# JoHof/lungmask

Measured on AMD Instinct MI355X. Metric: CT slices/sec (whole node), R231 512x512 volume, higher is better.
Workload: dtype f16x3-split (hi/lo f16 operands, f32 accumulate; fp32-class)

## Files before the change

### lungmask_amd/csrc/lm_platform.h

```cpp
#pragma once
#ifdef LM_EMU_BUILD
#include "hip_emu.h"
#else
#include <hip/hip_runtime.h>
#define LM_LAUNCH(kernel, grid, block, smem, stream, ...) \
    hipLaunchKernelGGL(kernel, (grid), (block), (smem), (stream), __VA_ARGS__)
#define LM_DYN_SMEM(name) extern __shared__ __attribute__((aligned(16))) char name[]
typedef float lm_f32x16 __attribute__((ext_vector_type(16)));
typedef float lm_f32x4 __attribute__((ext_vector_type(4)));
#endif
#include <cstdint>
#ifdef LM_EMU_BUILD
#define LM_IS_GPU_BUILD 0
#else
#define LM_IS_GPU_BUILD 1
#endif

#ifndef LM_EMU_BUILD
typedef _Float16 lm_h16;
typedef _Float16 lm_h16x8 __attribute__((ext_vector_type(8)));
__device__ __forceinline__ float lm_h2f(lm_h16 h) { return (float)h; }
__device__ __forceinline__ lm_h16 lm_f2h(float f) { return (lm_h16)f; }
#endif

// ... 208 lines not shown
    lm_h16 l[4] = {lm_f2h(v0 - lm_h2f(h[0])), lm_f2h(v1 - lm_h2f(h[1])), lm_f2h(v2 - lm_h2f(h[2])), lm_f2h(v3 - lm_h2f(h[3]))};
    memcpy(hi, h, 8);
    memcpy(lo, l, 8);
#else
    typedef _Float16 h4 __attribute__((ext_vector_type(4)));
    typedef float f4 __attribute__((ext_vector_type(4)));
    const f4 v = {v0, v1, v2, v3};
    const h4 h = __builtin_convertvector(v, h4);
    __builtin_memcpy(hi, &h, 8);
    unsigned l01, l23;
    asm("v_fma_mixlo_f16 %0, %1, 1.0, -%2 op_sel_hi:[0,0,1]" : "=v"(l01) : "v"(v0), "v"(hi->x));
    asm("v_fma_mixhi_f16 %0, %1, 1.0, -%2 op_sel:[0,0,1] op_sel_hi:[0,0,1]" : "+v"(l01) : "v"(v1), "v"(hi->x));
    asm("v_fma_mixlo_f16 %0, %1, 1.0, -%2 op_sel_hi:[0,0,1]" : "=v"(l23) : "v"(v2), "v"(hi->y));
    asm("v_fma_mixhi_f16 %0, %1, 1.0, -%2 op_sel:[0,0,1] op_sel_hi:[0,0,1]" : "+v"(l23) : "v"(v3), "v"(hi->y));
    lo->x = l01;
    lo->y = l23;
#endif
}
__device__ __forceinline__ unsigned lm_pk_absmax_u16(unsigned acc, unsigned two_halves) {
    const unsigned m = two_halves & 0x7fff7fffu;
#ifdef LM_EMU_BUILD
    const unsigned lo = (acc & 0xffffu) > (m & 0xffffu) ? (acc & 0xffffu) : (m & 0xffffu);
    const unsigned hi = (acc >> 16) > (m >> 16) ? (acc >> 16) : (m >> 16);
    return lo | (hi << 16);
#else
    typedef unsigned short u16x2 __attribute__((ext_vector_type(2)));
    u16x2 a, b;
    __builtin_memcpy(&a, &acc, 4);
    __builtin_memcpy(&b, &m, 4);
    a = __builtin_elementwise_max(a, b);
    unsigned r;
    __builtin_memcpy(&r, &a, 4);
    return r;
#endif
}
__device__ __forceinline__ bool lm_pk_out_of_f16_guard(unsigned acc) { return (acc & 0xffffu) >= 0x7800u || (acc >> 16) >= 0x7800u; }

__device__ __forceinline__ void lm_unsplit4(uint2 hi, uint2 lo, float* out) {
#ifdef LM_EMU_BUILD
    lm_h16 h[4], l[4];
    memcpy(h, &hi, 8);
    memcpy(l, &lo, 8);
    for (int k = 0; k < 4; ++k) out[k] = lm_h2f(l[k]) + lm_h2f(h[k]);
#else
    typedef _Float16 h4 __attribute__((ext_vector_type(4)));
    typedef float f4 __attribute__((ext_vector_type(4)));
    h4 h, l;
    __builtin_memcpy(&h, &hi, 8);
    __builtin_memcpy(&l, &lo, 8);
    const f4 r = __builtin_convertvector(l, f4) + __builtin_convertvector(h, f4);
    out[0] = r[0];
    out[1] = r[1];
    out[2] = r[2];
    out[3] = r[3];
#endif
}

#ifdef LM_EMU_BUILD
typedef float lm_f32x2 __attribute__((vector_size(8)));
#else
typedef float lm_f32x2 __attribute__((ext_vector_type(2)));
#endif

template <int K>
__device__ __forceinline__ void lm_fmac_rowbcast(float& acc, float w, float x) {
#ifdef LM_EMU_BUILD
    acc = fmaf(__shfl(w, ((int)(lm_emu::linear_tid() & 63) & ~15) | K), x, acc);
#else
    asm("v_fmac_f32_dpp %0, %1, %2 row_newbcast:%3 row_mask:0xf bank_mask:0xf" : "+v"(acc) : "v"(w), "v"(x), "n"(K));
#endif
}
template <int K>
__device__ __forceinline__ float lm_mov_rowbcast(float w) {
#ifdef LM_EMU_BUILD
    return __shfl(w, ((int)(lm_emu::linear_tid() & 63) & ~15) | K);
#else
    float r = 0.f;
    asm("v_mov_b32_dpp %0, %1 row_newbcast:%2 row_mask:0xf bank_mask:0xf" : "+v"(r) : "v"(w), "n"(K));
    return r;
#endif
}

#ifdef LM_EMU_BUILD
#define LM_SCHED_FENCE() \
    do {                 \
    } while (0)
#else
#define LM_SCHED_FENCE() __builtin_amdgcn_sched_barrier(0)
#endif
#ifdef LM_EMU_BUILD
#define LM_LDS_WAIT6(N, a, b, c, d, e, f) \
    do {                                  \
    } while (0)
#define LM_LDS_READ128(dst, ptr, OFF) (dst) = *reinterpret_cast<const lm_h16x8*>(reinterpret_cast<const char*>(ptr) + (OFF))
#define LM_LDS_WAIT8(N, a, b, c, d, e, f, g, h) \
    do {                                        \
    } while (0)
#define LM_LDS_WAIT5(N, a, b, c, d, e) \
    do {                               \
    } while (0)
#define LM_LDS_WAIT2(N, a, b) \
    do {                      \
    } while (0)
#define LM_LDS_WAIT1(N, a) \
    do {                   \
    } while (0)
#define LM_LDS_WRITE2_64(ptr, lo8, hi8)                                  \
    do {                                                                 \
        *reinterpret_cast<uint2*>(reinterpret_cast<char*>(ptr)) = (lo8); \
        *reinterpret_cast<uint2*>(reinterpret_cast<char*>(ptr) + 16) = (hi8); \
    } while (0)
#else
typedef unsigned lm_u32x2 __attribute__((ext_vector_type(2)));
#define LM_LDS_WRITE2_64(ptr, lo8, hi8)                                                                                      \
    do {                                                                                                                     \
        const lm_u32x2 d0_ = {(lo8).x, (lo8).y}, d1_ = {(hi8).x, (hi8).y};                                                   \
        asm volatile("ds_write2_b64 %0, %1, %2 offset1:2"                                                                    \
                     :                                                                                                       \
                     : "v"((unsigned)(size_t)(__attribute__((address_space(3))) char*)(ptr)), "v"(d0_), "v"(d1_)            \
                     : "memory");                                                                                            \
    } while (0)
#define LM_LDS_WAIT2(N, a, b)                                                                \
    do {                                                                                     \
        asm volatile("s_waitcnt lgkmcnt(%2)" : "+v"(a), "+v"(b) : "i"(N) : "memory");        \
        __builtin_amdgcn_sched_barrier(0);                                                   \
    } while (0)
#define LM_LDS_WAIT1(N, a)                                                                   \
    do {                                                                                     \
        asm volatile("s_waitcnt lgkmcnt(%1)" : "+v"(a) : "i"(N) : "memory");                 \
        __builtin_amdgcn_sched_barrier(0);                                                   \
    } while (0)
#define LM_LDS_WAIT5(N, a, b, c, d, e)                                                                            \
    do {                                                                                                          \
        asm volatile("s_waitcnt lgkmcnt(%5)" : "+v"(a), "+v"(b), "+v"(c), "+v"(d), "+v"(e) : "i"(N) : "memory");  \
        __builtin_amdgcn_sched_barrier(0);                                                                        \
    } while (0)
#define LM_LDS_WAIT6(N, a, b, c, d, e, f)                                                                         \
    do {                                                                                                          \
        asm volatile("s_waitcnt lgkmcnt(%6)" : "+v"(a), "+v"(b), "+v"(c), "+v"(d), "+v"(e), "+v"(f) : "i"(N) : "memory"); \
        __builtin_amdgcn_sched_barrier(0);                                                                        \
    } while (0)
#define LM_LDS_READ128(dst, ptr, OFF)                                                                             \
    asm volatile("ds_read_b128 %0, %1 offset:%2"                                                                  \
                 : "=v"(dst)                                                                                      \
                 : "v"((unsigned)(size_t)(__attribute__((address_space(3))) const char*)(ptr)), "i"(OFF)          \
                 : "memory")
#define LM_LDS_WAIT8(N, a, b, c, d, e, f, g, h)                                                                   \
    do {                                                                                                          \
        asm volatile("s_waitcnt lgkmcnt(%8)"                                                                      \
                     : "+v"(a), "+v"(b), "+v"(c), "+v"(d), "+v"(e), "+v"(f), "+v"(g), "+v"(h)                     \
                     : "i"(N)                                                                                     \
                     : "memory");                                                                                 \
        __builtin_amdgcn_sched_barrier(0);                                                                        \
    } while (0)
#endif
```

### lungmask_amd/csrc/nn_kernels_h3.hip

```cpp
#include <cstdlib>

#include "nn_kernels.h"

#if defined(LM_H3_TRACE) || defined(LM_H3_TIMELINE)
__device__ unsigned* lm_h3_trace_ptr = nullptr;
#endif

namespace lm {

namespace {

constexpr int TH = 16, TW = 16, TN = 64, KC = 16;

typedef uint2 __attribute__((may_alias)) uint2_a;
typedef uint4 __attribute__((may_alias)) uint4_a;

__device__ __forceinline__ void split_store4(char* group_base, int half_off_bytes, float v0, float v1, float v2, float v3) {
    uint2 ph, plo;
    lm_split4(v0, v1, v2, v3, &ph, &plo);
    *reinterpret_cast<uint2*>(group_base + half_off_bytes) = ph;
    *reinterpret_cast<uint2*>(group_base + 16 + half_off_bytes) = plo;
}

template <int TAPS>
struct H3Smem {
    static constexpr int HALO = (TAPS == 9) ? 1 : 0;
    static constexpr int PW = TW + 2 * HALO, PH = TH + 2 * HALO;
    static constexpr int A_ROWS = PH * PW;
    static constexpr int W_ROWS = TAPS * TN;
    static constexpr int ROW_BYTES = KC * 4;
    static constexpr int A_BYTES = ((A_ROWS * ROW_BYTES + 1023) / 1024) * 1024;
    static constexpr int W_BYTES = W_ROWS * ROW_BYTES;
    static constexpr int BYTES = A_BYTES + W_BYTES;
};

}

template <int TAPS>
__global__ __launch_bounds__(256, 2) void conv_igemm_h3(ConvParamsH3 p) {
    using SM = H3Smem<TAPS>;
    constexpr int HALO = SM::HALO, PW = SM::PW, A_ROWS = SM::A_ROWS, W_ROWS = SM::W_ROWS;
    LM_DYN_SMEM(smem);
    char* As = smem;
    char* Ws = smem + SM::A_BYTES;

    const int tid = threadIdx.x, lane = tid & 63, wave = tid >> 6;
    const int tiles_x = (p.W + TW - 1) / TW, tiles_y = (p.H + TH - 1) / TH;
    int t = blockIdx.x;
    const int tx = t % tiles_x;
    t /= tiles_x;
    const int ty = t % tiles_y;
    const int b = t / tiles_y;
    const int x0 = tx * TW, y0 = ty * TH, n0 = blockIdx.y * TN;

    lm_f32x16 accm[2][2];
#pragma unroll
    for (int i = 0; i < 2; ++i)
#pragma unroll
        for (int j = 0; j < 2; ++j)
#pragma unroll
            for (int r = 0; r < 16; ++r) {
                accm[i][j][r] = 0.f;
            }

    const int li = lane & 31, kb = lane >> 5;
    const int pr = li >> 4, pc = li & 15;
    const char* __restrict__ in_b = p.in + ((size_t)b * p.H * p.W * p.in_cstride + p.in_coff) * 4;
    const size_t w_row_bytes = (size_t)p.Cin * 4;

    for (int c0 = 0; c0 < p.Cin; c0 += KC) {
        __syncthreads();
        for (int piece = wave; piece * 64 < A_ROWS * 4; piece += 4) {
            const int idx = piece * 64 + lane;
            if (idx < A_ROWS * 4) {
                const int row = idx >> 2, ls = (idx & 3) ^ ((row >> 2) & 3);
                const int py = row / PW, px = row - py * PW;
                const int gy = y0 + py - HALO, gx = x0 + px - HALO;
                const char* src = p.zeros;
                if (gy >= 0 && gy < p.H && gx >= 0 && gx < p.W)
                    src = in_b + ((size_t)gy * p.W + gx) * p.in_cstride * 4 + (size_t)((c0 >> 3) + (ls >> 1)) * 32 + (ls & 1) * 16;
                lm_global_load_lds16(src, As + piece * 1024);
            }
        }
// ... 30 lines not shown
                for (int nt = 0; nt < 2; ++nt) {
                    accm[mt][nt] = lm_mfma_f32_32x32x16_f16(whi[mt], ahi[nt], accm[mt][nt]);
                    accm[mt][nt] = lm_mfma_f32_32x32x16_f16(whi[mt], alo[nt], accm[mt][nt]);
                    accm[mt][nt] = lm_mfma_f32_32x32x16_f16(wlo[mt], ahi[nt], accm[mt][nt]);
                }
        }
    }

    const bool bn = p.bn_s != nullptr;
    float amax = 0.f;
    const int Hp = p.H >> 1, Wp = p.W >> 1;
#pragma unroll
    for (int nt = 0; nt < 2; ++nt) {
        const int y = y0 + 4 * wave + 2 * nt + pr, x = x0 + pc;
        const bool inside = y < p.H && x < p.W;
        char* orow = p.out + ((((size_t)b * p.H + y) * p.W + x) * p.out_cstride + p.out_coff) * 4;
        const bool pool_lane = p.pool != nullptr && pr == 0 && (pc & 1) == 0;
        char* prow = p.pool ? p.pool + ((((size_t)b * Hp + (y >> 1)) * Wp + (x >> 1)) * p.pool_cstride + p.pool_coff) * 4 : nullptr;
#pragma unroll
        for (int mt = 0; mt < 2; ++mt) {
#pragma unroll
            for (int g = 0; g < 4; ++g) {
                const int cb = n0 + 32 * mt + 8 * g + 4 * kb;
                float4 bias = *reinterpret_cast<const float4*>(p.bias + cb);
                if (TAPS == 9 && p.border_corr != nullptr) {
                    const int mask = (y == 0 ? 1 : 0) | (y == p.H - 1 ? 2 : 0) | (x == 0 ? 4 : 0) | (x == p.W - 1 ? 8 : 0);
                    const float4 c = *reinterpret_cast<const float4*>(p.border_corr + (size_t)mask * p.Cout + cb);
                    bias.x -= c.x;
                    bias.y -= c.y;
                    bias.z -= c.z;
                    bias.w -= c.w;
                }
                float v[4];
                v[0] = fmaf(accm[mt][nt][4 * g + 0], p.acc_scale, bias.x);
                v[1] = fmaf(accm[mt][nt][4 * g + 1], p.acc_scale, bias.y);
                v[2] = fmaf(accm[mt][nt][4 * g + 2], p.acc_scale, bias.z);
                v[3] = fmaf(accm[mt][nt][4 * g + 3], p.acc_scale, bias.w);
                if (bn) {
                    const float4 s = *reinterpret_cast<const float4*>(p.bn_s + cb);
                    const float4 sh = *reinterpret_cast<const float4*>(p.bn_t + cb);
                    v[0] = fmaf(fmaxf(v[0], 0.f), s.x, sh.x);
                    v[1] = fmaf(fmaxf(v[1], 0.f), s.y, sh.y);
                    v[2] = fmaf(fmaxf(v[2], 0.f), s.z, sh.z);
                    v[3] = fmaf(fmaxf(v[3], 0.f), s.w, sh.w);
                }
                amax = fmaxf(fmaxf(amax, fabsf(v[0])), fmaxf(fmaxf(fabsf(v[1]), fabsf(v[2])), fabsf(v[3])));
                const int grp = cb >> 3;
                if (inside) split_store4(orow + (size_t)grp * 32, (cb & 7) * 2, v[0], v[1], v[2], v[3]);
                if (p.pool != nullptr) {
                    float q[4];
#pragma unroll
                    for (int k = 0; k < 4; ++k) {
                        const float h = v[k] + __shfl_xor(v[k], 1);
                        q[k] = 0.25f * (h + __shfl_xor(h, 16));
                    }
                    if (pool_lane && y + 1 < p.H && x + 1 < p.W) split_store4(prow + (size_t)grp * 32, (cb & 7) * 2, q[0], q[1], q[2], q[3]);
                }
            }
        }
    }
    if (p.range_flag != nullptr && !(amax < kF16Guard)) atomicOr(p.range_flag, 1u);
}

namespace {
template <int TAPS, bool G16>
struct H3WSmem {
    static constexpr int HALO = (TAPS == 9) ? 1 : 0;
    static constexpr int TWW = G16 ? 16 : 32;
    static constexpr int NSL = G16 ? 2 : 1;
    static constexpr int PW = TWW + 2 * HALO, PH = TH + 2 * HALO;
    static constexpr int SL_ROWS = PH * PW;
    static constexpr int A_ROWS = NSL * SL_ROWS;
    static constexpr int NTSTEP = G16 ? 2 : 1;
    static constexpr int W_ROWS = TAPS * TN;
    static constexpr int A_PIECES = (A_ROWS * 4 + 63) / 64, W_PIECES = W_ROWS * 4 / 64;
    static constexpr int A_BYTES = A_PIECES * 1024, W_BYTES = W_PIECES * 1024;
    static constexpr int BUF_BYTES = A_BYTES + W_BYTES;
    static constexpr int NW = 8;
    static constexpr int A_PER_WAVE = (A_PIECES + NW - 1) / NW, W_PER_WAVE = (W_PIECES + NW - 1) / NW;
};

__device__ __forceinline__ float4 as_float4(const lm_h16x8& v) {
    float4 r;
    memcpy(&r, &v, 16);
    return r;
}
}

#define H3P_READS(F, AS, DY, DX)                                                              \
    do {                                                                                      \
        const int a_lo_ = a_off[DX] ^ 16;                                                     \
        LM_LDS_READ128(F[4], (AS) + a_off[DX], (DY) * ROWB);                                  \
        LM_LDS_READ128(F[5], (AS) + a_lo_, (DY) * ROWB);                                      \
        LM_LDS_READ128(F[6], (AS) + a_off[DX], ((DY) + NTSTEP) * ROWB);                       \
        LM_LDS_READ128(F[7], (AS) + a_lo_, ((DY) + NTSTEP) * ROWB);                           \
        LM_LDS_READ128(F[0], (AS) + w_off, (3 * (DY) + (DX)) * (TN * 64));                    \
        LM_LDS_READ128(F[1], (AS) + w_off, (3 * (DY) + (DX)) * (TN * 64) + 2048);             \
        LM_LDS_READ128(F[2], (AS) + w_off_lo, (3 * (DY) + (DX)) * (TN * 64));                 \
        LM_LDS_READ128(F[3], (AS) + w_off_lo, (3 * (DY) + (DX)) * (TN * 64) + 2048);          \
    } while (0)
#define H3P_MFMA3(F, I0, I1, I2)                                                              \
    do {                                                                                      \
        H3P_MFMA1(F, I0);                                                                     \
        H3P_MFMA1(F, I1);                                                                     \
        H3P_MFMA1(F, I2);                                                                     \
    } while (0)
#define H3P_MFMA1(F, I)                                                                                                           \
    accm[((I) >> 1) & 1][(I) & 1] = lm_mfma_f32_32x32x16_f16(F[((I) < 8 ? 0 : 2) + (((I) >> 1) & 1)],                             \
                                                            F[4 + 2 * ((I) & 1) + (((I) >> 2) == 1 ? 1 : 0)], accm[((I) >> 1) & 1][(I) & 1])
#define H3P_MFMA2(F, I0, I1) \
    do {                     \
        H3P_MFMA1(F, I0);    \
        H3P_MFMA1(F, I1);    \
    } while (0)
#define H3P_MFMAS(F, PS)       \
    do {                       \
        prod_step(PS, 0);      \
        H3P_MFMA2(F, 0, 1);    \
        prod_step(PS, 1);      \
        H3P_MFMA2(F, 2, 3);    \
        prod_step(PS, 2);      \
        H3P_MFMA2(F, 4, 5);    \
        prod_step(PS, 3);      \
        H3P_MFMA2(F, 6, 7);    \
        prod_step(PS, 4);      \
        H3P_MFMA2(F, 8, 9);    \
        prod_step(PS, 5);      \
        H3P_MFMA2(F, 10, 11);  \
    } while (0)
#define H3P_MFMAS_D(F, K0, PS) \
    do {                       \
        prod_step(PS, 0);      \
        H3P_MFMA2(F, 0, 1);    \
        prod_step(PS, 1);      \
        H3P_MFMA1(F, 2);       \
        dma_slot((K0) + 0);    \
        H3P_MFMA1(F, 3);       \
        prod_step(PS, 2);      \
        H3P_MFMA2(F, 4, 5);    \
        dma_slot((K0) + 1);    \
        prod_step(PS, 3);      \
        H3P_MFMA2(F, 6, 7);    \
        prod_step(PS, 4);      \
        H3P_MFMA1(F, 8);       \
        dma_slot((K0) + 2);    \
        H3P_MFMA1(F, 9);       \
        prod_step(PS, 5);      \
        H3P_MFMA2(F, 10, 11);  \
        dma_slot((K0) + 3);    \
    } while (0)
#define H3P_WAITF(N, F) LM_LDS_WAIT8(N, F[0], F[1], F[2], F[3], F[4], F[5], F[6], F[7])
#define H3P_STEP(FC, FN, AS, NDY, NDX, PS) \
    do {                                   \
        H3P_READS(FN, AS, NDY, NDX);       \
        H3P_WAITF(8, FC);                  \
        H3P_MFMAS(FC, PS);                 \
    } while (0)
#define H3P_STEP_D(FC, FN, AS, NDY, NDX, K0, PS) \
    do {                                         \
        H3P_READS(FN, AS, NDY, NDX);             \
        H3P_WAITF(8, FC);                        \
        H3P_MFMAS_D(FC, K0, PS);                 \
    } while (0)
#define H3P_CHUNK_STEPS(FA, FB, AS)             \
    do {                                        \
        H3P_STEP_D(FA, FB, AS, 0, 1, 0, 1);     \
        H3P_STEP_D(FB, FA, AS, 0, 2, 4, 2);     \
        H3P_STEP_D(FA, FB, AS, 1, 0, 8, 3);     \
        H3P_STEP(FB, FA, AS, 1, 1, 4);          \
        H3P_STEP(FA, FB, AS, 1, 2, 5);          \
        H3P_STEP(FB, FA, AS, 2, 0, 6);          \
        H3P_STEP(FA, FB, AS, 2, 1, 7);          \
        H3P_STEP(FB, FA, AS, 2, 2, 8);          \
    } while (0)

#define H3P_EPI_READS(E, CL) LM_LDS_READ128(E[0], ep + (CL) * 4, 0)
#define H3P_EPI_WAIT(NEXT, E) LM_LDS_WAIT1((NEXT) ? 1 : 0, E[0])
#define H3P_EPI_CL(MG) (32 * ((MG) >> 2) + 8 * ((MG) & 3) + 4 * kb)

namespace {
constexpr int FC_PW = 36, FC_PH = 20, FC_PATCH = FC_PW * FC_PH;
constexpr int FC_CONST = 9 * 64 + 64 + 64;
constexpr int FC_ROW = 68;
static_assert(10 * FC_ROW <= FC_CONST, "the DPP producer's constant table");
constexpr int FC_TASKS = 18 * 34 * 2;

}

template <int TAPS, bool G16, int HEAD = 0, int PROD = 0, bool KS = false>
__global__ __launch_bounds__(512) void conv_igemm_h3p(ConvParamsH3 p, int n_ptiles, int n_items, int xcd_order) {
    using SM = H3WSmem<TAPS, G16>;
    static_assert(!KS || (TAPS == 9 && HEAD == 0 && PROD == 0), "the split-K instantiation is the plain 3x3 form");
    constexpr bool KSPLIT = TAPS == 1 || KS;
    static_assert(PROD == 0 || (TAPS == 9 && !G16 && HEAD == 0), "the loader-side producers belong to the 32-wide 3x3 form");
    constexpr int HALO = SM::HALO, PW = SM::PW, TWW = SM::TWW, NW = SM::NW, ROWB = PW * 64, NTSTEP = SM::NTSTEP;
    constexpr int ASWZ = (G16 && TAPS == 9) ? 1 : 2;
    constexpr int HSTR = 144;
    constexpr int STAGE_BYTES = NW * 64 * HSTR;
    constexpr int SUB = TAPS == 1 ? 2 : 1;
    constexpr int STAGE_EXTRA = STAGE_BYTES <= SUB * SM::BUF_BYTES ? 0 : STAGE_BYTES;
    __shared__ __attribute__((aligned(1024))) char lds[2 * SUB * SM::BUF_BYTES + STAGE_EXTRA];
    __shared__ __attribute__((aligned(16))) float epi[2][3][TN];
    __shared__ __attribute__((aligned(16))) float hw[HEAD ? kMaxClasses * 64 + kMaxClasses : 4];
    __shared__ __attribute__((aligned(16))) float fcx[PROD == 1 ? 2 * FC_PATCH : 4];
    __shared__ __attribute__((aligned(16))) float fcc[PROD == 1 ? FC_CONST : 4];

    const int tid = threadIdx.x, lane = tid & 63, wave = lm_uniform(tid >> 6);
    const int li = lane & 31, kb = lane >> 5;
    const int wsl = G16 ? (wave >> 2) : 0;
    const int wrow = G16 ? 4 * (wave & 3) + (li >> 4) : 2 * wave;
    const int wcol = G16 ? (li & 15) : li;

    int a_off[TAPS == 9 ? 3 : 1];
#pragma unroll
    for (int dx = 0; dx < (TAPS == 9 ? 3 : 1); ++dx) {
        const int px = wcol + dx;
        a_off[dx] = (wsl * SM::SL_ROWS + wrow * PW + px) * 64 + ((2 * kb) ^ ((px >> ASWZ) & 3)) * 16;
    }
    const int w_off = SM::A_BYTES + li * 64 + ((2 * kb) ^ ((li >> 2) & 3)) * 16;
    const int w_off_lo = w_off ^ 16;

    unsigned relA[SM::A_PER_WAVE];
    int pyx[SM::A_PER_WAVE];
#pragma unroll
    for (int j = 0; j < SM::A_PER_WAVE; ++j) {
        const int piece = wave + NW * j, idx = piece * 64 + lane;
        pyx[j] = -1;
        relA[j] = 0;
        if (PROD != 1 && piece < SM::A_PIECES && idx < SM::A_ROWS * 4) {
            const int row = idx >> 2;
            const int sl = row / SM::SL_ROWS, rr = row - sl * SM::SL_ROWS;
            const int py = rr / PW, px = rr - py * PW;
            const int ls = (idx & 3) ^ ((px >> ASWZ) & 3);
            relA[j] = (unsigned)(((sl * p.H + py) * p.W + px) * p.in_cstride * 4 + (ls >> 1) * 32 + (ls & 1) * 16);
            pyx[j] = py | (px << 8) | (sl << 16);
        }
    }
    unsigned voffW;
    {
        const int idx = wave * 64 + lane;
        const int row = idx >> 2, ls = (idx & 3) ^ ((row >> 2) & 3);
        const int tap = row / TN, n = row - tap * TN;
        voffW = (unsigned)((tap * p.Cout + n) * p.Cin * 4 + (ls >> 1) * 32 + (ls & 1) * 16);
    }
    const unsigned w_piece_stride = (unsigned)(NW * 64 / 4 / TN) * (unsigned)p.Cout * (unsigned)p.Cin * 4u;
    const unsigned slice_bytes = (unsigned)p.H * (unsigned)p.W * (unsigned)p.in_cstride * 4u;
    const lm_rsrc rsrcA = PROD == 1 ? lm_make_rsrc(p.fc_x, (size_t)p.B * p.H * p.W * 4)
                                    : lm_make_rsrc(p.in + (size_t)p.in_coff * 4, (size_t)p.B * slice_bytes - (size_t)p.in_coff * 4);
    const lm_rsrc rsrcW = lm_make_rsrc(p.w, (size_t)TAPS * p.Cout * p.Cin * 4);
    const int tiles_x = p.W / TWW;
    const int nchunks = p.Cin / KC / ((KSPLIT && p.ksplit > 1) ? p.ksplit : 1);
    constexpr bool bn = TAPS == 9;

    const int n_ct = p.Cout / TN;
    const int tiles_y = (p.H + TH - 1) / TH;
    const bool pow2 = ((n_ct & (n_ct - 1)) | (tiles_x & (tiles_x - 1)) | (tiles_y & (tiles_y - 1))) == 0;
    const int sh_ct = 31 - __clz(n_ct), sh_tx = 31 - __clz(tiles_x), sh_ty = 31 - __clz(tiles_y);
    const int ksplit = (KSPLIT && p.ksplit > 1) ? p.ksplit : 1;
    auto decode = [&](int it, int& b, int& y0, int& x0, int& n0, int& kc) -> bool {
        int ct, pt;
        if (xcd_order) {
// ... 333 lines not shown
                        } else {
                            H3P_EPI_WAIT(false, ec[mg & 1]);
                        }
                        const float4 bias = as_float4(ec[mg & 1][0]);
                        float bb[4] = {bias.x, bias.y, bias.z, bias.w};
                        if (border) {
                            const float4 c = cb[mg];
                            bb[0] -= c.x;
                            bb[1] -= c.y;
                            bb[2] -= c.z;
                            bb[3] -= c.w;
                        }
                        float v[4];
#pragma unroll
                        for (int k = 0; k < 4; ++k) {
                            float t = fmaf(accm[mt][nt][4 * g4 + k], p.acc_scale, bb[k]);
                            if (bn) t = fmaxf(t, 0.f);
                            v[k] = t;
                        }
#pragma unroll
                        for (int k = 0; k < 4; ++k) vv[mg][k] = v[k];
                    }
                    float best = 0.f;
                    int arg = 0;
                    float lgs[HEAD == 2 ? kMaxClasses : 1];
                    auto logit = [&](int c) __attribute__((always_inline)) -> float {
                        float sq[8];
#pragma unroll
                        for (int q = 0; q < 8; ++q) {
                            const float4 w4 = *reinterpret_cast<const float4*>(&hw[c * 64 + 8 * q + 4 * kb]);
                            float s0 = fmaf(vv[q][0], w4.x, 0.f);
                            s0 = fmaf(vv[q][1], w4.y, s0);
                            s0 = fmaf(vv[q][2], w4.z, s0);
                            s0 = fmaf(vv[q][3], w4.w, s0);
                            float s1 = __shfl_xor(s0, 32);
                            s1 = fmaf(vv[q][0], w4.x, s1);
                            s1 = fmaf(vv[q][1], w4.y, s1);
                            s1 = fmaf(vv[q][2], w4.z, s1);
                            s1 = fmaf(vv[q][3], w4.w, s1);
                            sq[q] = s1;
                        }
                        return (((sq[0] + sq[4]) + (sq[2] + sq[6])) + ((sq[1] + sq[5]) + (sq[3] + sq[7]))) + hw[kMaxClasses * 64 + c];
                    };
                    if constexpr (HEAD == 2) {
#pragma unroll
                        for (int c = 0; c < kMaxClasses; ++c) {
                            if (c < p.head_C) {
                                const float lg = logit(c);
                                lgs[c] = lg;
                                if (c == 0 || lg > best) {
                                    best = lg;
                                    arg = c;
                                }
                            }
                        }
                    } else {
#pragma unroll 1
                        for (int c = 0; c < p.head_C; ++c) {
                            const float lg = logit(c);
                            if (c == 0 || lg > best) {
                                best = lg;
                                arg = c;
                            }
                        }
                    }
                    if (tile_ok && kb == 1) p.head_labels[((size_t)bs * p.H + yl) * p.W + x0 + li] = (uint8_t)arg;
                    if constexpr (HEAD == 2) {
                        float se = 0.f;
#pragma unroll
                        for (int c = 0; c < kMaxClasses; ++c)
                            if (c < p.head_C) se += expf(lgs[c] - best);
                        const float lse = best + logf(se);
                        if (tile_ok && kb == 1) {
                            const size_t HW = (size_t)p.H * p.W, yx = (size_t)yl * p.W + x0 + li;
#pragma unroll
                            for (int c = 0; c < kMaxClasses; ++c)
                                if (c < p.head_C) p.head_logp[((size_t)bs * p.head_C + c) * HW + yx] = lgs[c] - lse;
                        }
                    }
                }
            } else {
            int yl2[2], bmask2[2];
            bool ok2[2], border2[2];
            char* obase[2];
#pragma unroll
            for (int nt = 0; nt < 2; ++nt) {
                yl2[nt] = G16 ? yb + 2 * nt + (li >> 4) : yb + nt;
                ok2[nt] = bs < p.B && (G16 ? yb + 2 * nt + 1 < p.H : yb + nt < p.H);
                const int xl = G16 ? wcol : x0 + li;
                bmask2[nt] = (yl2[nt] == 0 ? 1 : 0) | (yl2[nt] == p.H - 1 ? 2 : 0) | (xl == 0 ? 4 : 0) | (xl == p.W - 1 ? 8 : 0);
                border2[nt] = TAPS == 9 && p.border_corr != nullptr && __any(bmask2[nt] != 0);
                const int y_first = G16 ? yb + 2 * nt : yb + nt;
                obase[nt] = p.out + ((((size_t)bs * p.H + y_first) * p.W + x0) * p.out_cstride + p.out_coff + n0) * 4;
            }
#pragma unroll
            for (int mt = 0; mt < 2; ++mt) {
                float4 cb[2][2];
                auto load_cb = [&](int g4) __attribute__((always_inline)) {
#pragma unroll
                    for (int nt = 0; nt < 2; ++nt)
                        if (border2[nt])
                            cb[g4 & 1][nt] = *reinterpret_cast<const float4*>(p.border_corr + (size_t)bmask2[nt] * p.Cout + n0 + H3P_EPI_CL(4 * mt + g4));
                };
                load_cb(0);
                float qs[4][4];
                lm_h16x8 ec[2][3];
                H3P_EPI_READS(ec[0], H3P_EPI_CL(4 * mt));
#pragma unroll
                for (int g4 = 0; g4 < 4; ++g4) {
                    const int mg = 4 * mt + g4;
                    const int cl = H3P_EPI_CL(mg);
                    if (g4 + 1 < 4) {
                        H3P_EPI_READS(ec[(g4 + 1) & 1], H3P_EPI_CL(mg + 1));
                        H3P_EPI_WAIT(true, ec[g4 & 1]);
                    } else {
                        H3P_EPI_WAIT(false, ec[g4 & 1]);
                    }
                    const float4 bias = as_float4(ec[g4 & 1][0]);
                    if (g4 + 1 < 4) load_cb(g4 + 1);
                    float v[2][4];
#pragma unroll
                    for (int nt = 0; nt < 2; ++nt) {
                        float bb[4] = {bias.x, bias.y, bias.z, bias.w};
                        if (border2[nt]) {
                            const float4 c = cb[g4 & 1][nt];
                            bb[0] -= c.x;
                            bb[1] -= c.y;
                            bb[2] -= c.z;
                            bb[3] -= c.w;
                        }
#pragma unroll
                        for (int k = 0; k < 4; ++k) {
                            float t = fmaf(accm[mt][nt][4 * g4 + k], p.acc_scale, bb[k]);
                            if (bn) t = fmaxf(t, 0.f);
                            v[nt][k] = t;
                        }
                        uint2 ph, plo;
                        lm_split4(v[nt][0], v[nt][1], v[nt][2], v[nt][3], &ph, &plo);
                        gmax = lm_pk_absmax_u16(lm_pk_absmax_u16(gmax, ph.x), ph.y);
                        char* d = hstage + (nt * 32 + li) * HSTR + ((cl & 31) >> 3) * 32 + (cl & 7) * 2;
                        *reinterpret_cast<uint2_a*>(d) = ph;
                        *reinterpret_cast<uint2_a*>(d + 16) = plo;
                        if (G16 && p.pool != nullptr) {
                            float q[4];
#pragma unroll
                            for (int k = 0; k < 4; ++k) {
                                const float h = v[nt][k] + __shfl_xor(v[nt][k], 16);
                                q[k] = 0.25f * (h + __shfl_xor(h, 1));
                            }
                            if (ok2[nt] && (li & 17) == 0) {
                                const int cg = n0 + cl;
                                char* prow = p.pool + ((((size_t)bs * Hp + (yl2[nt] >> 1)) * Wp + (wcol >> 1)) * p.pool_cstride + p.pool_coff) * 4;
                                split_store4(prow + (size_t)(cg >> 3) * 32, (cg & 7) * 2, q[0], q[1], q[2], q[3]);
                            }
                        }
                    }
                    if (!G16 && p.pool != nullptr) {
#pragma unroll
                        for (int k = 0; k < 4; ++k) {
                            const float pl = v[0][k] + v[1][k];
                            qs[g4][k] = 0.25f * (pl + lm_lane_xor1(pl));
                        }
                    }
                }
                LM_TRACE_SUB(5);
                lm_wave_lds_fence();
#pragma unroll
                for (int i = 0; i < 8; ++i) {
                    const int q = i * 64 + lane, px = q >> 3, part = q & 7;
                    if (ok2[i >> 2]) {
                        const uint4 val = *reinterpret_cast<const uint4_a*>(hstage + px * HSTR + part * 16);
                        char* dst = obase[i >> 2] + (size_t)(px & 31) * p.out_cstride * 4 + mt * 128 + part * 16;
                        if (p.stream_out) lm_store16_stream(dst, val);
                        else *reinterpret_cast<uint4_a*>(dst) = val;
                    }
                }
                lm_wave_lds_fence();
                LM_TRACE_SUB(6);
                if (!G16 && p.pool != nullptr) {
#pragma unroll
                    for (int g4 = 0; g4 < 4; ++g4) {
                        const int cl = H3P_EPI_CL(4 * mt + g4);
                        uint2 ph, plo;
                        lm_split4(qs[g4][0], qs[g4][1], qs[g4][2], qs[g4][3], &ph, &plo);
                        if ((li & 1) == 0) {
                            char* d = hstage + (li >> 1) * HSTR + ((cl & 31) >> 3) * 32 + (cl & 7) * 2;
                            *reinterpret_cast<uint2_a*>(d) = ph;
                            *reinterpret_cast<uint2_a*>(d + 16) = plo;
                        }
                    }
                    lm_wave_lds_fence();
                    if (bs < p.B && yb + 1 < p.H) {
                        char* prow = p.pool + ((((size_t)bs * Hp + (yb >> 1)) * Wp + (x0 >> 1)) * p.pool_cstride + p.pool_coff + n0) * 4;
#pragma unroll
                        for (int i = 0; i < 2; ++i) {
                            const int q = i * 64 + lane, px = q >> 3, part = q & 7;
                            const uint4 val = *reinterpret_cast<const uint4_a*>(hstage + px * HSTR + part * 16);
                            *reinterpret_cast<uint4_a*>(prow + (size_t)px * p.pool_cstride * 4 + mt * 128 + part * 16) = val;
                        }
                    }
                    lm_wave_lds_fence();
                }
            }
            }
            if (p.range_flag != nullptr && lm_pk_out_of_f16_guard(gmax)) atomicOr(p.range_flag, 1u);
        }
        LM_TRACE_MARK(3);
        if (!have_next) break;
        it = nit;
        b = nb;
        y0 = ny0;
        x0 = nx0;
        n0 = nn0;
        kc0 = nkc0;
#pragma unroll
        for (int j = 0; j < SM::A_PER_WAVE; ++j) voffC[j] = voffN[j];
        epar ^= 1;
        lm_barrier_lds();
        LM_TRACE_MARK(4);
    }
    if (PROD != 0 && p.range_flag != nullptr && lm_pk_out_of_f16_guard(pr_max)) atomicOr(p.range_flag, 1u);
    LM_TRACE_FLUSH();
}

static bool h3_persistent_ok(const ConvParamsH3& p, int taps) {
    static const bool wide_ok = [] { const char* e = getenv("LM_H3_FALLBACK"); return !(e && e[0] == '1'); }();
    const size_t slice_bytes = (size_t)p.H * p.W * p.in_cstride * 4;
    return wide_ok && (p.W % 32 == 0 || p.W == 16) && (p.Cin / KC) % (taps == 1 ? 4 : 2) == 0 && 2 * slice_bytes < 0x7fffffffull &&
           (size_t)taps * p.Cout * p.Cin * 4 < 0x7fffffffull && (p.bn_s != nullptr) == (taps == 9);
}

template <int TAPS>
static hipError_t launch_conv_h3_t(const ConvParamsH3& p, hipStream_t stream) {
    if (p.Cin % KC != 0 || p.Cout % TN != 0 || (p.in_cstride & 7) || (p.in_coff & 7) || (p.out_cstride & 7) || (p.out_coff & 7)) return hipErrorInvalidValue;
    if (p.pool != nullptr && (((p.H | p.W) & 1) || (p.pool_cstride & 7) || (p.pool_coff & 7))) return hipErrorInvalidValue;
    if (h3_persistent_ok(p, TAPS)) {
        const bool g16 = p.W == 16;
        static const int order_env = [] { const char* e = getenv("LM_H3_ORDER"); return e ? atoi(e) : -1; }();
        static const int n_cu = [] {
            int dev = 0, n = 256;
            if (hipGetDevice(&dev) == hipSuccess) (void)hipDeviceGetAttribute(&n, hipDeviceAttributeMultiprocessorCount, dev);
            return n > 0 ? n : 256;
        }();
        const size_t slice_bytes = (size_t)p.H * p.W * p.in_cstride * 4;
        const int max_b = std::max(2, (int)(0x7fffffffull / slice_bytes) & ~1);
        for (int b0 = 0; b0 < p.B; b0 += max_b) {
            ConvParamsH3 pd = p;
            pd.B = std::min(max_b, p.B - b0);
            pd.in = p.in + (size_t)b0 * slice_bytes;
            pd.out = p.out + (size_t)b0 * p.H * p.W * p.out_cstride * 4;
            if (p.pool) pd.pool = p.pool + (size_t)b0 * (p.H / 2) * (p.W / 2) * p.pool_cstride * 4;
            if (p.head_labels) pd.head_labels = p.head_labels + (size_t)b0 * p.H * p.W;
            if (p.head_logp) pd.head_logp = p.head_logp + (size_t)b0 * p.head_C * p.H * p.W;
            if (p.fc_x) pd.fc_x = p.fc_x + (size_t)b0 * p.H * p.W;
            const int n_ptiles = g16 ? ((p.H + TH - 1) / TH) * ((pd.B + 1) / 2) : (p.W / 32) * ((p.H + TH - 1) / TH) * pd.B;
            const int n_ct = p.Cout / TN;
            const int ks = p.ksplit > 1 ? p.ksplit : 1;
            const int xcd_order = ks > 1 ? 0 : (order_env >= 0 ? order_env : (n_ct >= 2 && n_ptiles >= 64 ? 1 : 0));
            const int n_items = xcd_order ? 8 * ((n_ptiles + 7) / 8) * n_ct : n_ptiles * n_ct * ks;
            const unsigned blocks = (unsigned)std::min(n_items, n_cu);
            if (TAPS == 9 && ks > 1) {
                if (g16) LM_LAUNCH((conv_igemm_h3p<9, true, 0, 0, true>), dim3(blocks), dim3(512), 0, stream, pd, n_ptiles, n_items, xcd_order);
                else LM_LAUNCH((conv_igemm_h3p<9, false, 0, 0, true>), dim3(blocks), dim3(512), 0, stream, pd, n_ptiles, n_items, xcd_order);
            } else if (g16)
                LM_LAUNCH((conv_igemm_h3p<TAPS, true>), dim3(blocks), dim3(512), 0, stream, pd, n_ptiles, n_items, xcd_order);
            else if (TAPS == 9 && pd.head_labels != nullptr && pd.head_logp != nullptr)
                LM_LAUNCH((conv_igemm_h3p<9, false, 2>), dim3(blocks), dim3(512), 0, stream, pd, n_ptiles, n_items, xcd_order);
            else if (TAPS == 9 && pd.head_labels != nullptr)
                LM_LAUNCH((conv_igemm_h3p<9, false, 1>), dim3(blocks), dim3(512), 0, stream, pd, n_ptiles, n_items, xcd_order);
            else if (TAPS == 9 && pd.fc_x != nullptr)
                LM_LAUNCH((conv_igemm_h3p<9, false, 0, 1>), dim3(blocks), dim3(512), 0, stream, pd, n_ptiles, n_items, xcd_order);
            else
                LM_LAUNCH((conv_igemm_h3p<TAPS, false>), dim3(blocks), dim3(512), 0, stream, pd, n_ptiles, n_items, xcd_order);
            const hipError_t err = hipGetLastError();
            if (err != hipSuccess) return err;
        }
        return hipSuccess;
    }
    const int tiles = ((p.W + TW - 1) / TW) * ((p.H + TH - 1) / TH);
    dim3 grid((unsigned)(tiles * p.B), (unsigned)(p.Cout / TN));
    LM_LAUNCH((conv_igemm_h3<TAPS>), grid, dim3(256), (H3Smem<TAPS>::BYTES), stream, p);
    return hipGetLastError();
}

bool conv3x3_h3_can_fuse_head(const ConvParamsH3& p) {
// ... 361 lines not shown
```

Before: 4479.

## Batch epilogue LDS reads and hoist border-correction and pool stores out of loop

Restructures the conv epilogue. The output write-back now issues eight ds_read_b128 up front with explicit partial lgkmcnt waits and uses precomputed per-lane row pointers. The stream/non-stream choice is resolved at compile time instead of per store. Border-correction vectors are loaded once for all 8 channel groups before the mt loop, and the pooled-output staging/store is merged into a single pass after both mt iterations. This cuts LDS latency stalls, per-iteration global loads and address arithmetic, at the cost of more live registers (cb[8][2], qs[8][4]), which may lower occupancy or cause spills.

```diff
diff --git a/lungmask_amd/csrc/lm_platform.h b/lungmask_amd/csrc/lm_platform.h
--- a/lungmask_amd/csrc/lm_platform.h
+++ b/lungmask_amd/csrc/lm_platform.h
@@ -314,6 +314,13 @@
 }
 
 #ifdef LM_EMU_BUILD
+#define LM_ASM_TAG(T) \
+    do {              \
+    } while (0)
+#else
+#define LM_ASM_TAG(T) asm volatile("; " T ::: "memory")
+#endif
+#ifdef LM_EMU_BUILD
 #define LM_SCHED_FENCE() \
     do {                 \
     } while (0)
@@ -330,6 +337,9 @@
     } while (0)
 #define LM_LDS_WAIT5(N, a, b, c, d, e) \
     do {                               \
+    } while (0)
+#define LM_LDS_WAIT4(N, a, b, c, d) \
+    do {                            \
     } while (0)
 #define LM_LDS_WAIT2(N, a, b) \
     do {                      \
@@ -361,6 +371,11 @@
     do {                                                                                     \
         asm volatile("s_waitcnt lgkmcnt(%1)" : "+v"(a) : "i"(N) : "memory");                 \
         __builtin_amdgcn_sched_barrier(0);                                                   \
+    } while (0)
+#define LM_LDS_WAIT4(N, a, b, c, d)                                                                               \
+    do {                                                                                                          \
+        asm volatile("s_waitcnt lgkmcnt(%4)" : "+v"(a), "+v"(b), "+v"(c), "+v"(d) : "i"(N) : "memory");           \
+        __builtin_amdgcn_sched_barrier(0);                                                                        \
     } while (0)
 #define LM_LDS_WAIT5(N, a, b, c, d, e)                                                                            \
     do {                                                                                                          \
diff --git a/lungmask_amd/csrc/nn_kernels_h3.hip b/lungmask_amd/csrc/nn_kernels_h3.hip
--- a/lungmask_amd/csrc/nn_kernels_h3.hip
+++ b/lungmask_amd/csrc/nn_kernels_h3.hip
@@ -1,4 +1,5 @@
 #include <cstdlib>
+#include <type_traits>
 
 #include "nn_kernels.h"
 
@@ -195,6 +196,11 @@
 
 __device__ __forceinline__ float4 as_float4(const lm_h16x8& v) {
     float4 r;
+    memcpy(&r, &v, 16);
+    return r;
+}
+__device__ __forceinline__ uint4 as_uint4(const lm_h16x8& v) {
+    uint4 r;
     memcpy(&r, &v, 16);
     return r;
 }
@@ -290,6 +296,8 @@
 #define H3P_EPI_READS(E, CL) LM_LDS_READ128(E[0], ep + (CL) * 4, 0)
 #define H3P_EPI_WAIT(NEXT, E) LM_LDS_WAIT1((NEXT) ? 1 : 0, E[0])
 #define H3P_EPI_CL(MG) (32 * ((MG) >> 2) + 8 * ((MG) & 3) + 4 * kb)
+#define H3P_OUT_READ(L, BASE, I) LM_LDS_READ128(L[I], BASE, (I) * 8 * HSTR)
+#define H3P_OUT_WAIT4(N, L, I) LM_LDS_WAIT4(N, L[(I)], L[(I) + 1], L[(I) + 2], L[(I) + 3])
 
 namespace {
 constexpr int FC_PW = 36, FC_PH = 20, FC_PATCH = FC_PW * FC_PH;
@@ -789,7 +797,7 @@
             } else {
             int yl2[2], bmask2[2];
             bool ok2[2], border2[2];
-            char* obase[2];
+            char* orow[2];
 #pragma unroll
             for (int nt = 0; nt < 2; ++nt) {
                 yl2[nt] = G16 ? yb + 2 * nt + (li >> 4) : yb + nt;
@@ -798,19 +806,63 @@
                 bmask2[nt] = (yl2[nt] == 0 ? 1 : 0) | (yl2[nt] == p.H - 1 ? 2 : 0) | (xl == 0 ? 4 : 0) | (xl == p.W - 1 ? 8 : 0);
                 border2[nt] = TAPS == 9 && p.border_corr != nullptr && __any(bmask2[nt] != 0);
                 const int y_first = G16 ? yb + 2 * nt : yb + nt;
-                obase[nt] = p.out + ((((size_t)bs * p.H + y_first) * p.W + x0) * p.out_cstride + p.out_coff + n0) * 4;
-            }
+                orow[nt] = p.out + ((((size_t)bs * p.H + y_first) * p.W + x0 + (lane >> 3)) * p.out_cstride + p.out_coff + n0) * 4 + (lane & 7) * 16;
+            }
+            const size_t ostep = (size_t)p.out_cstride * 32;
+            const char* const hread = hstage + (lane >> 3) * HSTR + (lane & 7) * 16;
+            lm_f32x4 cb[TAPS == 9 ? 8 : 1][2];
+            if constexpr (TAPS == 9) {
+                if (border2[0] || border2[1]) {
+#pragma unroll
+                    for (int mg = 0; mg < 8; ++mg)
+#pragma unroll
+                        for (int nt = 0; nt < 2; ++nt)
+                            cb[mg][nt] = *reinterpret_cast<const lm_f32x4*>(p.border_corr + (size_t)bmask2[nt] * p.Cout + n0 + H3P_EPI_CL(mg));
+#pragma unroll
+                    for (int mg = 0; mg < 8; ++mg)
+#pragma unroll
+                        for (int nt = 0; nt < 2; ++nt) LM_PIN(cb[mg][nt]);
+                } else {
+#pragma unroll
+                    for (int mg = 0; mg < 8; ++mg)
+#pragma unroll
+                        for (int nt = 0; nt < 2; ++nt) cb[mg][nt] = lm_f32x4{0.f, 0.f, 0.f, 0.f};
+                }
+            }
+            auto store_lines = [&](int mt, auto stream) __attribute__((always_inline)) {
+                lm_h16x8 ln[8];
+                LM_ASM_TAG("LM_STORE_OUT_BEGIN");
+                H3P_OUT_READ(ln, hread, 0);
+                H3P_OUT_READ(ln, hread, 1);
+                H3P_OUT_READ(ln, hread, 2);
+                H3P_OUT_READ(ln, hread, 3);
+                H3P_OUT_READ(ln, hread, 4);
+                H3P_OUT_READ(ln, hread, 5);
+                H3P_OUT_READ(ln, hread, 6);
+                H3P_OUT_READ(ln, hread, 7);
+                H3P_OUT_WAIT4(4, ln, 0);
+                if (ok2[0]) {
+#pragma unroll
+                    for (int i = 0; i < 4; ++i) {
+                        char* dst = orow[0] + i * ostep + mt * 128;
+                        if constexpr (decltype(stream)::value) lm_store16_stream(dst, as_uint4(ln[i]));
+                        else *reinterpret_cast<uint4_a*>(dst) = as_uint4(ln[i]);
+                    }
+                }
+                H3P_OUT_WAIT4(0, ln, 4);
+                if (ok2[1]) {
+#pragma unroll
+                    for (int i = 0; i < 4; ++i) {
+                        char* dst = orow[1] + i * ostep + mt * 128;
+                        if constexpr (decltype(stream)::value) lm_store16_stream(dst, as_uint4(ln[4 + i]));
+                        else *reinterpret_cast<uint4_a*>(dst) = as_uint4(ln[4 + i]);
+                    }
+                }
+                LM_ASM_TAG("LM_STORE_OUT_END");
+            };
+            float qs[8][4];
 #pragma unroll
             for (int mt = 0; mt < 2; ++mt) {
-                float4 cb[2][2];
-                auto load_cb = [&](int g4) __attribute__((always_inline)) {
-#pragma unroll
-                    for (int nt = 0; nt < 2; ++nt)
-                        if (border2[nt])
-                            cb[g4 & 1][nt] = *reinterpret_cast<const float4*>(p.border_corr + (size_t)bmask2[nt] * p.Cout + n0 + H3P_EPI_CL(4 * mt + g4));
-                };
-                load_cb(0);
-                float qs[4][4];
                 lm_h16x8 ec[2][3];
                 H3P_EPI_READS(ec[0], H3P_EPI_CL(4 * mt));
 #pragma unroll
@@ -824,17 +876,16 @@
                         H3P_EPI_WAIT(false, ec[g4 & 1]);
                     }
                     const float4 bias = as_float4(ec[g4 & 1][0]);
-                    if (g4 + 1 < 4) load_cb(g4 + 1);
                     float v[2][4];
 #pragma unroll
                     for (int nt = 0; nt < 2; ++nt) {
                         float bb[4] = {bias.x, bias.y, bias.z, bias.w};
-                        if (border2[nt]) {
-                            const float4 c = cb[g4 & 1][nt];
-                            bb[0] -= c.x;
-                            bb[1] -= c.y;
-                            bb[2] -= c.z;
-                            bb[3] -= c.w;
+                        if constexpr (TAPS == 9) {
+                            const lm_f32x4 c = cb[mg][nt];
+                            bb[0] -= c[0];
+                            bb[1] -= c[1];
+                            bb[2] -= c[2];
+                            bb[3] -= c[3];
                         }
 #pragma unroll
                         for (int k = 0; k < 4; ++k) {
@@ -855,6 +906,8 @@
                                 const float h = v[nt][k] + __shfl_xor(v[nt][k], 16);
                                 q[k] = 0.25f * (h + __shfl_xor(h, 1));
                             }
+#pragma unroll
+                            for (int k = 0; k < 4; ++k) LM_PIN(q[k]);
                             if (ok2[nt] && (li & 17) == 0) {
                                 const int cg = n0 + cl;
                                 char* prow = p.pool + ((((size_t)bs * Hp + (yl2[nt] >> 1)) * Wp + (wcol >> 1)) * p.pool_cstride + p.pool_coff) * 4;
@@ -866,48 +919,46 @@
 #pragma unroll
                         for (int k = 0; k < 4; ++k) {
                             const float pl = v[0][k] + v[1][k];
-                            qs[g4][k] = 0.25f * (pl + lm_lane_xor1(pl));
+                            qs[mg][k] = 0.25f * (pl + lm_lane_xor1(pl));
                         }
                     }
                 }
                 LM_TRACE_SUB(5);
                 lm_wave_lds_fence();
-#pragma unroll
-                for (int i = 0; i < 8; ++i) {
-                    const int q = i * 64 + lane, px = q >> 3, part = q & 7;
-                    if (ok2[i >> 2]) {
-                        const uint4 val = *reinterpret_cast<const uint4_a*>(hstage + px * HSTR + part * 16);
-                        char* dst = obase[i >> 2] + (size_t)(px & 31) * p.out_cstride * 4 + mt * 128 + part * 16;
-                        if (p.stream_out) lm_store16_stream(dst, val);
-                        else *reinterpret_cast<uint4_a*>(dst) = val;
-                    }
-                }
+                if (p.stream_out) store_lines(mt, std::true_type{});
+                else store_lines(mt, std::false_type{});
                 lm_wave_lds_fence();
                 LM_TRACE_SUB(6);
-                if (!G16 && p.pool != nullptr) {
-#pragma unroll
-                    for (int g4 = 0; g4 < 4; ++g4) {
-                        const int cl = H3P_EPI_CL(4 * mt + g4);
-                        uint2 ph, plo;
-                        lm_split4(qs[g4][0], qs[g4][1], qs[g4][2], qs[g4][3], &ph, &plo);
-                        if ((li & 1) == 0) {
-                            char* d = hstage + (li >> 1) * HSTR + ((cl & 31) >> 3) * 32 + (cl & 7) * 2;
-                            *reinterpret_cast<uint2_a*>(d) = ph;
-                            *reinterpret_cast<uint2_a*>(d + 16) = plo;
-                        }
+            }
+            if (!G16 && p.pool != nullptr) {
+#pragma unroll
+                for (int mg = 0; mg < 8; ++mg) {
+                    const int cl = H3P_EPI_CL(mg);
+                    uint2 ph, plo;
+                    lm_split4(qs[mg][0], qs[mg][1], qs[mg][2], qs[mg][3], &ph, &plo);
+                    if ((li & 1) == 0) {
+                        char* d = hstage + ((mg >> 2) * 16 + (li >> 1)) * HSTR + ((cl & 31) >> 3) * 32 + (cl & 7) * 2;
+                        *reinterpret_cast<uint2_a*>(d) = ph;
+                        *reinterpret_cast<uint2_a*>(d + 16) = plo;
                     }
-                    lm_wave_lds_fence();
-                    if (bs < p.B && yb + 1 < p.H) {
-                        char* prow = p.pool + ((((size_t)bs * Hp + (yb >> 1)) * Wp + (x0 >> 1)) * p.pool_cstride + p.pool_coff + n0) * 4;
-#pragma unroll
-                        for (int i = 0; i < 2; ++i) {
-                            const int q = i * 64 + lane, px = q >> 3, part = q & 7;
-                            const uint4 val = *reinterpret_cast<const uint4_a*>(hstage + px * HSTR + part * 16);
-                            *reinterpret_cast<uint4_a*>(prow + (size_t)px * p.pool_cstride * 4 + mt * 128 + part * 16) = val;
-                        }
-                    }
-                    lm_wave_lds_fence();
-                }
+                }
+                lm_wave_lds_fence();
+                lm_h16x8 ln[4];
+                LM_ASM_TAG("LM_STORE_OUT_BEGIN");
+                H3P_OUT_READ(ln, hread, 0);
+                H3P_OUT_READ(ln, hread, 1);
+                H3P_OUT_READ(ln, hread, 2);
+                H3P_OUT_READ(ln, hread, 3);
+                H3P_OUT_WAIT4(0, ln, 0);
+                if (bs < p.B && yb + 1 < p.H) {
+                    char* prow = p.pool + ((((size_t)bs * Hp + (yb >> 1)) * Wp + (x0 >> 1) + (lane >> 3)) * p.pool_cstride + p.pool_coff + n0) * 4 + (lane & 7) * 16;
+                    const size_t pstep = (size_t)p.pool_cstride * 32;
+#pragma unroll
+                    for (int i = 0; i < 4; ++i)
+                        *reinterpret_cast<uint4_a*>(prow + (i & 1) * pstep + (i >> 1) * 128) = as_uint4(ln[i]);
+                }
+                LM_ASM_TAG("LM_STORE_OUT_END");
+                lm_wave_lds_fence();
             }
             }
             if (p.range_flag != nullptr && lm_pk_out_of_f16_guard(gmax)) atomicOr(p.range_flag, 1u);
```

After: 4521 (median of 6 runs). Within noise of the previous version (+0.9%).
